# peterWon/LVI-ExC

Measured on AMD Instinct MI355X. Metric: M residual+Jacobian evals/s per GN iter, higher is better.
Workload: dtype f64; 1 GPU; config4-full-LVI: 1000000 surfel + 200000 IMU samples (gyro+accel blocks) + 49992 ORB reprojection blocks, 25023 knots @ dt=0.02; step = residuals + analytic Jacobians + Huber + J^T J/J^T r assembly (no linear solve); n_tangent=155259, bandwidth=179, n_border=52, tracks=orb, parallelism=sequence-per-gpu x1, allreduce_transport=none (one sequence)

## Files before the change

lvi-exc_amd/csrc/lvx_eval.hip:

```cpp
#include <algorithm>
#include <cmath>
#include <cstring>
#include <functional>
#include <numeric>
#include <cstdlib>

#include <thread>
#include "lvx_ctx.h"

namespace lvx {

#define LVX_PW 4
struct Keys { int k0, k1, lm; };
LVX_HD bool same(const Keys& a, const Keys& b) { return a.k0 == b.k0 && a.k1 == b.k1 && a.lm == b.lm; }

struct Cal { ImuCal imu; SensorCal lidar, cam; const double* rho; };
__device__ __forceinline__ Cal load_cal(const DevCommon& cm) {
  const double* s = cm.state + 7 * (size_t)cm.N;
  Cal c;
  c.imu.tau = s[7]; c.imu.roll = s[8]; c.imu.pitch = s[9]; c.imu.ba = load_v3(s + 10); c.imu.bg = load_v3(s + 13);
  c.lidar.q = load_q(s + 16); c.lidar.p = load_v3(s + 20); c.lidar.tau = s[23];
  c.cam.q = load_q(s + 24); c.cam.p = load_v3(s + 28); c.cam.tau = s[31];
  c.rho = s + 32;
  return c;
// ... 248 lines not shown
  double J[NR][NC];
  Keys key{-1, -1, -1};
  bool valid = false;
  if (in) {
    int status;
    if constexpr (EXP) status = eval_flat(fam, cm, sp, cal, hub, si, r, J, key);
    else status = fam.eval(cm, sp, cal, hub, si, r, J, key);
    valid = status == RES_OK;
    if (!valid) { atomicOr(cm.err, status); key = Keys{-1, -1, -1}; }
    if constexpr (EXP) {
      if (valid) put_record<NR, NC>(cm, F::FAM, fam.perm[si], key.k0, F::KEYS > 1 ? key.k1 : -1, F::KEYS > 2 ? key.lm : -1, [&](int a, int c) { return J[a][c]; });
      else put_skipped(cm, F::FAM, fam.perm[si]);
    }
  }
  double mycost = 0.0;
  if (valid) {
    double s = 0.0;
#pragma unroll
    for (int a = 0; a < NR; ++a) s += r[a] * r[a];
    double scale;
    mycost = 0.5 * huber_rho(fam.huber, s, &scale);
    const long long orow = row0 + (long long)fam.perm[si] * NR;
    if (cm.residuals) {
#pragma unroll
      for (int a = 0; a < NR; ++a) cm.residuals[orow + a] = r[a];
    }
    if (!EXP && cm.jcols) {
#pragma unroll
      for (int a = 0; a < NR; ++a) {
        int32_t* jc = cm.jcols + (orow + a) * LVX_JAC_WIDTH;
        double* jv = cm.jvals + (orow + a) * LVX_JAC_WIDTH;
#pragma unroll
        for (int c = 0; c < NC; ++c) {
          const int g = fam.col(c, key, cm.N);
          const bool dead = tangent_locked(g, cm.N, cm.L, cm.locks);
          jc[c] = dead ? -1 : g;
          jv[c] = dead ? 0.0 : J[a][c];
        }
        for (int c = NC; c < LVX_JAC_WIDTH; ++c) { jc[c] = -1; jv[c] = 0.0; }
      }
    }
    if (scale != 1.0) {
#pragma unroll
      for (int a = 0; a < NR; ++a) {
        r[a] *= scale;
#pragma unroll
        for (int c = 0; c < NC; ++c) J[a][c] *= scale;
      }
    }
  }
  mycost = wave_sum(mycost);
  if (lane == 0) atomicAdd(&cm.cost[rep], mycost);
  if (cm.what & LVX_EVAL_NORMAL_EQ) {
#pragma unroll
    for (int a = 0; a < NR; ++a) {
      rs[lane * NR + a] = valid ? r[a] : 0.0;
#pragma unroll
      for (int c = 0; c < NC; ++c) Jt[c * TS + lane * NR + a] = valid ? J[a][c] : 0.0;
    }
    Keys pk;
    pk.k0 = __shfl_up(key.k0, 1); pk.k1 = __shfl_up(key.k1, 1); pk.lm = __shfl_up(key.lm, 1);
    const bool head = (lane == 0) || !same(pk, key);
    const unsigned long long heads = __ballot(head);
    const int myseg = __popcll(heads & ((2ull << lane) - 1ull)) - 1;
    if (head) { seg_l0[myseg] = lane; seg_ok[myseg] = valid ? 1 : 0; seg_keys[myseg] = key; }
    if (lane == 0) nseg_s = __popcll(heads);
  }
  }
  if (!(cm.what & LVX_EVAL_NORMAL_EQ)) return;
  __syncthreads();
  const int nseg = nseg_s;
  const int tid = threadIdx.x;
  constexpr int NT = 64 * PW;
  for (int e = tid; e < nseg * NC; e += NT) { const int sg = e / NC, c = e % NC; cpos[e] = seg_ok[sg] ? cm.ord[fam.col(c, seg_keys[sg], cm.N)] : LVX_DEAD; }
  constexpr int ITER = (NP + NC + NT - 1) / NT;
  unsigned code[ITER];
#pragma unroll
  for (int i = 0; i < ITER; ++i) { const int p = tid + NT * i; code[i] = p < NP ? pairs[p] : 0u; }
  __syncthreads();
  for (int sg = 0; sg < nseg; ++sg) {
    if (!seg_ok[sg]) continue;
    const int l0 = seg_l0[sg];
    const int l1 = sg + 1 < nseg ? seg_l0[sg + 1] : 64;
    const int rb = l0 * NR, re = l1 * NR;
    const int* cp = &cpos[sg * NC];
#pragma unroll
    for (int i = 0; i < ITER; ++i) {
      const int p = tid + NT * i;
      if (p < NP) {
        const int a = code[i] & 0xff, b = code[i] >> 8;
        const int pa = cp[a], pb = cp[b];
        if (pa == LVX_DEAD || pb == LVX_DEAD) continue;
        const double* ja = &Jt[a * TS];
        const double* jb = &Jt[b * TS];
        double acc = 0.0;
        for (int row = rb; row < re; ++row) acc += ja[row] * jb[row];
        if (a != b && pa == pb) acc *= 2.0;
        add_H(cm, pa, pb, acc, rep);
      } else if (p < NP + NC) {
        const int c = p - NP;
        const int pc = cp[c];
        if (pc == LVX_DEAD) continue;
        const double* jc = &Jt[c * TS];
        double acc = 0.0;
        for (int row = rb; row < re; ++row) acc += jc[row] * rs[row];
        add_g(cm, pc, acc, rep);
      }
    }
  }
}

__device__ void hub_eval_thread(const DevCommon& cm, double t_map, int want_surf, int want_cs, HubShared* hubs, int s) {
  if (s > 1) return;
  if ((s == 0 && !want_surf) || (s == 1 && !want_cs)) { hubs[s].ok = 0; return; }
  const SplineRef sp{cm.t0, cm.dt, cm.N, cm.state, cm.state + 3 * (size_t)cm.N};
  const Cal cal = load_cal(cm);
  const bool tl = s == 0 ? (cm.locks & LVX_LOCK_LIDAR_TAU) != 0 : (cm.locks & LVX_LOCK_CAM_TAU) != 0;
  const double tau = s == 0 ? cal.lidar.tau : cal.cam.tau;
  double s1[1][2]; hub_spans(t_map, tl, cm.sensor_mto, s1);
  Segs sg; KnotRef kh; hubs[s].ok = 0;
  if (!build_segments(sp, s1, 1, &sg)) return;
  if (!seg_lookup(sp, sg, t_map + tau, &kh)) return;
  if (!(tl ? pose_eval<true>(sp, kh, &hubs[s].A) : pose_eval<true, true>(sp, kh, &hubs[s].A))) { hubs[s].ok = -RES_NONUNIT; return; }
  hub_matrix(hubs[s].A, hubs[s].M);
  hubs[s].ok = 1;
}
__device__ __forceinline__ void state_prepass_block(const DevCommon& cm, So3Pre* tab, int nblk_tab, double t_map, int want_surf, int want_cs, HubShared* hubs, int blk) {
  if (blk >= nblk_tab) { hub_eval_thread(cm, t_map, want_surf, want_cs, hubs, threadIdx.x); return; }
  const int k = blk * blockDim.x + threadIdx.x;
  if (k >= cm.N) return;
  const double* so3 = cm.state + 3 * (size_t)cm.N;
  So3Pre e;
  if (k + 1 < cm.N) so3_pre(load_q(so3 + 4 * (size_t)k), load_q(so3 + 4 * (size_t)(k + 1)), &e);
  else { e.Om = mk(0, 0, 0); e.on = 0.0; e.Jri = m3_identity(); e.c3 = 1.0 / 12.0; e.ok = 1; }
  tab[k] = e;
}

struct Aux { int wid, xk, lm; const PreWin* pw; };
struct GyroAcc {
  enum { PMAJ = 1 };
  enum { NK = 12, NG = 3, NR = 3, HUB = -1, KPK = 3, LVO = 3, WS = 1, GL = 32, SKIP_GG = 0, SECONDARY = 0, LB = 64, NCP = 15, USE_PRE = 1, OCC = 1, FAM = LVX_FAM_GYRO };
  __device__ static constexpr int jm(int c) { return c; }
  int n; const double* t; const double* m3; const int* perm; double weight, huber;
  __device__ int eval(const DevCommon& cm, const SplineRef& sp, const Cal& cal, const HubShared*, int si, double r[NR], double (*J)[NCP], int& key, Aux& aux) const {
    return gyro_residual<true, true>(sp, cal.imu, t[si], load_v3(m3 + 3 * (size_t)si), weight, &key, r, J, aux.pw);
  }
  __device__ static int klv(int c) { return 6 * (c / 3) + 3 + c % 3; }
  __device__ static int gcol(int g, int N, int nt) { return 6 * N + 5 + g; }
  __device__ void put(const DevCommon& cm, const HubShared*, int si, bool valid, int key, const double (*J)[NCP]) const {
    if (!valid) { put_skipped(cm, FAM, perm[si]); return; }
    put_record<NR, GYRO_NC>(cm, FAM, perm[si], key, -1, -1, [&](int a, int c) { return J[a][c]; });
  }
};
template <bool TAU> struct SurfAccT {
  enum { NK = 24, NG = 12 + (TAU ? 1 : 0), NR = 1, HUB = 0, KPK = 6, LVO = 0, WS = 2, GL = 16, SKIP_GG = 0, SECONDARY = 0, LB = 64, NCP = 36 + (TAU ? 1 : 0), USE_PRE = 1, OCC = 2, FAM = LVX_FAM_SURFEL };
  __device__ static constexpr int jm(int c) { return c; }
  int n; const double* t; const double* pt; const double* rowpl; const int* perm; double t_map, weight, huber;
  struct Row { double t; v3 p, Pi; };
  enum { PREFETCH = 1 };
  __device__ Row load(int si) const { return Row{t[si], load_v3(pt + 3 * (size_t)si), load_v3(rowpl + 3 * (size_t)si)}; }
  __device__ int eval_row(const DevCommon& cm, const SplineRef& sp, const Cal& cal, const HubShared* hub, const Row& row, double r[NR], double (*J)[NCP], int& key, Aux& aux) const {
    const bool tl = (cm.locks & LVX_LOCK_LIDAR_TAU) != 0;
    const double tk = row.t;
    Segs segs;
    if (tl) {
      KnotRef kr;
      const int st = two_point_lookup(sp, t_map, tk, tk + cal.lidar.tau, &kr);
      if (st >= 0) {
        if (st == 1) return RES_RANGE;
        if (hub->ok != 1) return hub->ok < 0 ? RES_NONUNIT : RES_RANGE;
        if (st == 2) return RES_RANGE;
        LVX_KT(aux.pw, 8)
        return surfel_residual_pseudo<true, TAU>(sp, hub->A, segs, cal.lidar, tk, row.p, row.Pi, weight, &key, r, J, aux.pw, &kr);
      }
    }
    const double pad = tl ? 0.0 : cm.sensor_mto;
    const double spans[2][2] = {{t_map - pad, t_map + pad}, {tk - pad, tk + pad}};
    if (!build_segments(sp, spans, 2, &segs)) return RES_RANGE;
    KnotRef kh;
    if (!seg_lookup(sp, segs, t_map + cal.lidar.tau, &kh)) return RES_RANGE;
    if (hub->ok != 1) return hub->ok < 0 ? RES_NONUNIT : RES_RANGE;
    if (kh.i0 != hub->A.k.i0 || kh.u != hub->A.k.u) return LVX_ERR_FALLBACK;
    LVX_KT(aux.pw, 8)
    return surfel_residual_pseudo<true, TAU>(sp, hub->A, segs, cal.lidar, tk, row.p, row.Pi, weight, &key, r, J, aux.pw);
  }
  __device__ static int klv(int c) { return c; }
  __device__ static int gcol(int g, int N, int nt) { return g < 6 ? nt + g : 6 * N + 8 + (g - 6); }
  __device__ void put(const DevCommon& cm, const HubShared* hub, int si, bool valid, int key, const double (*J)[NCP]) const {
    if (!valid) { put_skipped(cm, FAM, perm[si]); return; }
    put_record<NR, SURF_NC + (TAU ? 1 : 0)>(cm, FAM, perm[si], hub->A.k.i0, key, -1, [&](int a, int c) { return c < 24 ? hub_col(*hub, &J[a][24], c) : (c < 48 ? J[a][c - 24] : J[a][c - 18]); });
  }
};
using SurfAcc = SurfAccT<false>;
template <bool TAU> struct CamSurfAccT {
  enum { NK = 24, NG = 18 + (TAU ? 1 : 0), NR = 1, HUB = 1, KPK = 6, LVO = 0, WS = 1, GL = 16, SKIP_GG = 0, SECONDARY = 0, LB = 64, NCP = 42 + (TAU ? 1 : 0), USE_PRE = 1, OCC = 2, FAM = LVX_FAM_CAMSURF };
  __device__ static constexpr int jm(int c) { return c; }
  int n; const int* lm; const int* plane; const int* perm; const double* planes; const double* lm_uv; const double* lm_t0; double t_map, weight, huber;
  __device__ int eval(const DevCommon& cm, const SplineRef& sp, const Cal& cal, const HubShared* hub, int si, double r[NR], double (*J)[NCP], int& key, Aux& aux) const {
    const bool tl = (cm.locks & LVX_LOCK_CAM_TAU) != 0;
    const int l = lm[si];
    const double tk = lm_t0[l];
    Segs segs;
    if (tl) {
      KnotRef kr;
      const int st = two_point_lookup(sp, t_map, tk, tk + cal.cam.tau, &kr);
      if (st >= 0) {
        if (st == 1) return RES_RANGE;
        if (hub->ok != 1) return hub->ok < 0 ? RES_NONUNIT : RES_RANGE;
        if (st == 2) return RES_RANGE;
        return camsurf_residual_pseudo<true, TAU>(sp, hub->A, segs, cm.cam, cal.cam, cal.lidar, lm_uv[2 * l], lm_uv[2 * l + 1], tk, cal.rho[l],
                                                  load_v3(planes + 3 * (size_t)plane[si]), weight, &key, r, J, aux.pw, &kr);
      }
    }
    const double pad = tl ? 0.0 : cm.sensor_mto;
    const double spans[2][2] = {{t_map - pad, t_map + pad}, {tk - pad, tk + pad}};
    if (!build_segments(sp, spans, 2, &segs)) return RES_RANGE;
    KnotRef kh;
    if (!seg_lookup(sp, segs, t_map + cal.cam.tau, &kh)) return RES_RANGE;
    if (hub->ok != 1) return hub->ok < 0 ? RES_NONUNIT : RES_RANGE;
    if (kh.i0 != hub->A.k.i0 || kh.u != hub->A.k.u) return LVX_ERR_FALLBACK;
    return camsurf_residual_pseudo<true, TAU>(sp, hub->A, segs, cm.cam, cal.cam, cal.lidar, lm_uv[2 * l], lm_uv[2 * l + 1], tk, cal.rho[l],
                                              load_v3(planes + 3 * (size_t)plane[si]), weight, &key, r, J, aux.pw);
  }
  __device__ static int klv(int c) { return c; }
  __device__ static int gcol(int g, int N, int nt) { return g < 6 ? nt + 6 + g : (g < 12 ? 6 * N + 15 + (g - 6) : (g < 18 ? 6 * N + 8 + (g - 12) : 6 * N + 21)); }
  __device__ void put(const DevCommon& cm, const HubShared* hub, int si, bool valid, int key, const double (*J)[NCP]) const {
    if (!valid) { put_skipped(cm, FAM, perm[si]); return; }
    put_record<NR, CS_NC + (TAU ? 1 : 0)>(cm, FAM, perm[si], hub->A.k.i0, key, -1, [&](int a, int c) { return c < 24 ? hub_col(*hub, &J[a][24], c) : (c < 48 ? J[a][c - 24] : J[a][c - 18]); });
  }
};
using CamSurfAcc = CamSurfAccT<false>;

struct RepJac { const double* J; const double* r; const int* k; int n; };
template <int SIDE, bool TAU = false> struct RepSideAcc {
  enum { PMAJ = 1 };
  enum { NK = 24, NG = 6 + (TAU ? 1 : 0), NR = 2, HUB = -1, KPK = 6, LVO = 0, WS = 1, GL = 16, SKIP_GG = SIDE, SECONDARY = 1, LB = 16, NCP = 31 + (TAU ? 1 : 0), USE_PRE = 0, OCC = 1, FAM = LVX_FAM_REPROJ };
  __device__ static constexpr int jm(int c) { return c; }
  static constexpr int RJ = REP_NC + (TAU ? 1 : 0);
  int n; RepJac jac;
  double huber;
  __device__ int eval(const DevCommon&, const SplineRef&, const Cal&, const HubShared*, int si, double r[NR], double (*J)[NCP], int& key, Aux& aux) const {
    const int k = jac.k[(size_t)SIDE * jac.n + si];
    if (jac.k[(size_t)jac.n + si] < 0) return -1;
    key = k; aux.wid = k;
#pragma unroll
    for (int a = 0; a < 2; ++a) {
      r[a] = jac.r[(size_t)a * jac.n + si];
#pragma unroll
      for (int c = 0; c < 24; ++c) J[a][c] = jac.J[(size_t)(a * RJ + 24 * SIDE + c) * jac.n + si];
#pragma unroll
      for (int c = 0; c < 6; ++c) J[a][24 + c] = jac.J[(size_t)(a * RJ + 48 + c) * jac.n + si];
      if (TAU) J[a][30] = jac.J[(size_t)(a * RJ + 55) * jac.n + si];
    }
    return RES_OK;
  }
  __device__ static int gcol(int g, int N, int nt) { return 6 * N + 15 + g; }
};

template <bool TAU, bool EXP = false>
__global__ __launch_bounds__(64) void k_reproj_jac(ReprojFamT<TAU> fam, DevCommon cm, double* Jb, double* rb, int* kb, long long row0, double* Trec) {
  constexpr int RJ = REP_NC + (TAU ? 1 : 0), RW = 56 + (TAU ? 1 : 0);
  constexpr int RS = RW | 1;
  extern __shared__ double trec_s[];
  const int lane = threadIdx.x, si = blockIdx.x * 64 + lane, n = fam.n;
  const int rep = blockIdx.x % cm.nrep;
  double mycost = 0.0;
  if (si < n) {
    const SplineRef sp{cm.t0, cm.dt, cm.N, cm.state, cm.state + 3 * (size_t)cm.N};
    const Cal cal = load_cal(cm);
    HubShared none;
    double r[2], J[2][RJ];
    Keys key{-1, -1, -1};
    const int status = fam.eval_pre(cm, sp, cal, si, r, J, key);
    if constexpr (EXP) {
      if (status != RES_OK) put_skipped(cm, LVX_FAM_REPROJ, fam.perm[si]);
      else put_record<2, RJ>(cm, LVX_FAM_REPROJ, fam.perm[si], key.k0, key.k1, key.lm, [&](int a, int c) { return J[a][c]; });
    }
    if (status != RES_OK) { if (status == RES_OUTSIDE) fallback_row(cm, LVX_FAM_REPROJ, si); else atomicOr(cm.err, status); kb[si] = -1; kb[n + si] = -1; }
    else {
      double scale;
      mycost = 0.5 * huber_rho(fam.huber, r[0] * r[0] + r[1] * r[1], &scale);
      if (cm.residuals) { const long long orow = row0 + (long long)fam.perm[si] * 2; cm.residuals[orow] = r[0]; cm.residuals[orow + 1] = r[1]; }
      kb[si] = key.k0; kb[n + si] = key.k1;
      if (cm.what & LVX_EVAL_NORMAL_EQ) {
#pragma unroll
        for (int a = 0; a < 2; ++a) {
          rb[(size_t)a * n + si] = r[a] * scale;
#pragma unroll
          for (int c = 0; c < RJ; ++c) Jb[(size_t)(a * RJ + c) * n + si] = J[a][c] * scale;
        }
        if (Trec) {
          double* rec = trec_s + lane * RS;
          const double j0 = J[0][54] * scale, j1 = J[1][54] * scale;
#pragma unroll
          for (int c = 0; c < 54; ++c) rec[c] = j0 * (J[0][c] * scale) + j1 * (J[1][c] * scale);
          rec[54] = j0 * j0 + j1 * j1;
          rec[55] = j0 * (r[0] * scale) + j1 * (r[1] * scale);
          if (TAU) rec[56] = j0 * (J[0][55] * scale) + j1 * (J[1][55] * scale);
        }
      }
    }
  }
  if (Trec && (cm.what & LVX_EVAL_NORMAL_EQ)) {
    __builtin_amdgcn_fence(__ATOMIC_RELEASE, "wavefront");
    __builtin_amdgcn_wave_barrier();
    __builtin_amdgcn_fence(__ATOMIC_ACQUIRE, "wavefront");
    const int nrec = min(64, n - (int)blockIdx.x * 64);
    double* dst = Trec + (size_t)blockIdx.x * 64 * RW;
// ... 193 lines not shown
      else if (status != RES_OK) atomicOr(cm.err, status);
      else {
        valid = true;
        double scale;
        mycost = 0.5 * huber_rho(fam.huber, r[0] * r[0] + r[1] * r[1], &scale);
        if (cm.residuals) { const long long orow = row0 + (long long)fam.perm[si] * 2; cm.residuals[orow] = r[0]; cm.residuals[orow + 1] = r[1]; }
        if (scale != 1.0) {
#pragma unroll
          for (int a = 0; a < 2; ++a) {
            r[a] *= scale;
#pragma unroll
            for (int c = 0; c < RJ; ++c) J[a][c] *= scale;
          }
        }
      }
    }
    mycost = wave_sum(mycost);
    if (lane == 0 && mycost != 0.0) atomicAdd(&cm.cost[rep], mycost);
#ifdef RF_EVAL_ONLY
    if (cm.N > 0) continue;
#endif
    if (!want_ne) continue;
    const int my_w0 = valid ? key.k0 >> 2 : -1, my_w1 = valid ? key.k1 >> 2 : -1;
    const int my_o0 = 6 * (key.k0 & 3), my_o1 = 48 + 6 * (key.k1 & 3);
    const int my_p0 = (valid && lm_free) ? cm.lm_p0[key.lm] : 0;
    unsigned long long rem = __ballot(valid);
    while (rem) {
      const int lf = __ffsll((long long)rem) - 1;
      const int w0 = __builtin_amdgcn_readfirstlane(__shfl(my_w0, lf)), w1 = __builtin_amdgcn_readfirstlane(__shfl(my_w1, lf));
      const unsigned long long wm = __ballot(valid && my_w0 == w0 && my_w1 == w1);
      rem &= ~wm;
      for (int c = lane; c < 96; c += 64) {
        int tg = -1;
        if (c < 42) { if (4 * w0 + c / 6 < N) tg = 24 * w0 + c; }
        else if (c < 48) tg = 6 * N + 15 + (c - 42);
        else if (c < 90) { if (4 * w1 + (c - 48) / 6 < N) tg = 24 * w1 + (c - 48); }
        else if (c == TCOL && TAU) tg = 6 * N + 21;
        posL[c] = tg >= 0 ? cm.ord[tg] : LVX_DEAD;
      }
      d4 D[21];
#pragma unroll
      for (int t = 0; t < 21; ++t) D[t] = d4{0.0, 0.0, 0.0, 0.0};
      unsigned long long todo = wm;
      while (todo) {
        const int l0 = __ffsll((long long)todo) - 1;
        const int ws = min(l0, 48);
        const unsigned long long chunk = todo & (0xffffull << ws);
        todo &= ~chunk;
        for (int e = lane; e < 32 * LDP; e += 64) P[e] = 0.0;
        __builtin_amdgcn_fence(__ATOMIC_RELEASE, "wavefront");
        __builtin_amdgcn_wave_barrier();
        if ((chunk >> lane) & 1ull) {
#pragma unroll
          for (int a = 0; a < 2; ++a) {
            double* prow_ = P + ((lane - ws) * 2 + a) * LDP;
#pragma unroll
            for (int c = 0; c < 24; ++c) prow_[my_o0 + c] = J[a][c];
#pragma unroll
            for (int c = 0; c < 6; ++c) prow_[42 + c] = J[a][48 + c];
#pragma unroll
            for (int c = 0; c < 24; ++c) prow_[my_o1 + c] = J[a][24 + c];
            if (TAU) prow_[TCOL] = J[a][RJ - 1];
            prow_[RCOL] = r[a];
            prow_[LCOL] = J[a][54];
          }
        }
        __builtin_amdgcn_fence(__ATOMIC_RELEASE, "wavefront");
        __builtin_amdgcn_wave_barrier();
        __builtin_amdgcn_fence(__ATOMIC_ACQUIRE, "wavefront");
#ifndef RF_NO_LM
        if (lm_free) {
          for (int e0 = 0; e0 < 16 * (LCOL + 1); e0 += 64) {
            const int e = e0 + lane;
            const int li = min(e / (LCOL + 1), 15), c = e - li * (LCOL + 1);
            const int src = ws + li;
            const int p0 = __shfl(my_p0, src), l = __shfl(key.lm, src);
            if (e >= 16 * (LCOL + 1) || !((chunk >> src) & 1ull)) continue;
            const double* ra = P + (2 * li) * LDP;
            const double v = ra[LCOL] * ra[c] + ra[LDP + LCOL] * ra[LDP + c];
            if (v == 0.0) continue;
            int slot;
            if (c == RCOL) slot = cm.lm_wl + cm.nbd + 1;
            else if (c == LCOL) slot = cm.lm_wl + cm.nbd;
            else {
              const int p = posL[c];
              if (p == LVX_DEAD) continue;
              if (p >= 0) { slot = p - p0; if (slot < 0 || slot >= cm.lm_wl) { atomicOr(cm.err, 4); continue; } }
              else slot = cm.lm_wl + (-1 - p);
            }
            atomicAdd(&cm.lmH[(size_t)l * cm.lm_ls + slot], v);
          }
        }
#endif
        const int lhi = 63 - __clzll((long long)chunk);
        const int ks0 = (l0 - ws) >> 1, ks1 = (2 * (lhi - ws + 1) + 3) >> 2;
#ifndef RF_NO_MFMA
        for (int ks = ks0; ks < ks1; ++ks) {
          double f[6];
          const double* src = P + (4 * ks + (lane >> 4)) * LDP + (lane & 15);
#pragma unroll
          for (int c = 0; c < 6; ++c) f[c] = src[c * 16];
          int t = 0;
#pragma unroll
          for (int ci = 0; ci < 6; ++ci)
#pragma unroll
            for (int cj = ci; cj < 6; ++cj, ++t) D[t] = __builtin_amdgcn_mfma_f64_16x16x4f64(f[ci], f[cj], D[t], 0, 0, 0);
        }
#endif
        __builtin_amdgcn_fence(__ATOMIC_RELEASE, "wavefront");
        __builtin_amdgcn_wave_barrier();
      }
#pragma unroll
      for (int h = 0; h < 2; ++h) {
#pragma unroll
        for (int t = 11 * h; t < (h ? 21 : 11); ++t)
#pragma unroll
          for (int v = 0; v < 4; ++v) P[(t - 11 * h) * 256 + ((lane >> 4) + 4 * v) * 16 + (lane & 15)] = D[t][v];
        __builtin_amdgcn_fence(__ATOMIC_RELEASE, "wavefront");
        __builtin_amdgcn_wave_barrier();
        __builtin_amdgcn_fence(__ATOMIC_ACQUIRE, "wavefront");
#ifndef RF_NO_FLUSH
        for (int ci = 0, t = 0; ci < 6; ++ci)
          for (int cj = ci; cj < 6; ++cj, ++t) {
            if (t / 11 != h) continue;
            for (int e = lane; e < 256; e += 64) {
              const int row = ci * 16 + (e >> 4), col = cj * 16 + (e & 15);
              const double val = P[(t - 11 * h) * 256 + e];
              if (val == 0.0 || col < row) continue;
              const int pa = posL[row], pb = posL[col];
              if (row == RCOL) { if (col != RCOL && pb != LVX_DEAD) add_g(cm, pb, val, rep); continue; }
              if (col == RCOL) { if (pa != LVX_DEAD) add_g(cm, pa, val, rep); continue; }
              if (pa == LVX_DEAD || pb == LVX_DEAD) continue;
              add_H(cm, pa, pb, (pa == pb && row != col) ? 2.0 * val : val, rep);
            }
          }
#endif
        __builtin_amdgcn_fence(__ATOMIC_RELEASE, "wavefront");
        __builtin_amdgcn_wave_barrier();
      }
    }
  }
}

#define ACC_BW 24


struct NoRow {};
template <class F, class = void> struct RowOf { using type = NoRow; static constexpr bool prefetch = false; };
template <class F> struct RowOf<F, std::void_t<typename F::Row>> { using type = typename F::Row; static constexpr bool prefetch = true; };

template <class F, class = void> struct PanelMajor { static constexpr bool on = false; };
template <class F> struct PanelMajor<F, std::enable_if_t<(F::PMAJ > 0)>> { static constexpr bool on = true; static_assert(F::WS == 1, "panel-major needs shift-free windows"); };

template <class F> struct MfmaGeom {
  static constexpr int NKL = (F::WS + 3) * F::KPK;
  static constexpr int NCL = NKL + F::NG + 1;
  static constexpr int NT = (NCL + 15) / 16;
  static constexpr int LDP = (NT * 16) | 1;
  static constexpr int PR = F::GL * F::NR;
  static_assert(PR % 4 == 0, "panel rows must be a multiple of the MFMA k-step");
  static constexpr int NTP = NT * (NT + 1) / 2;
};
template <class F> size_t mfma_lds_bytes(int cr) {
  const int LV = (cr + 5) * 6;
  return (size_t)(LV * ACC_BW + F::NG * LV + F::NG * F::NG + LV + F::NG + 64 + 4 * MfmaGeom<F>::PR * MfmaGeom<F>::LDP) * 8 + (F::USE_PRE ? (size_t)(cr + 4) * sizeof(So3Pre) : 0) +
         (size_t)(LV + F::NG) * 4 + 64;
}

template <class F, int OCC, bool EXP = false>
__global__ __launch_bounds__(256, OCC) void k_family_mfma(F fam, DevCommon cm, const int* __restrict__ chunk_off, long long row0, int CR, int var_nch, const int* __restrict__ det_list) {
  using G = MfmaGeom<F>;
  constexpr int NK = F::NK, NG = F::NG, NC = F::NCP, NR = F::NR, KPK = F::KPK, WS = F::WS, GL = F::GL, LB = F::LB;
  constexpr int NKL = G::NKL, NT = G::NT, LDP = G::LDP, PR = G::PR;
  const int ACC_LV = (CR + 5) * 6;
  extern __shared__ double sm[];
  double* acc_band = sm;
  double* acc_bd = acc_band + ACC_LV * ACC_BW;
  double* acc_gg = acc_bd + NG * ACC_LV;
  double* acc_gk = acc_gg + NG * NG;
  double* acc_gG = acc_gk + ACC_LV;
  const int dummy = (int)(acc_gG + NG - sm);
  double* panels = acc_gG + NG + 64;
  So3Pre* pre_tab = (So3Pre*)(panels + 4 * PR * LDP);
  int* kpos = (int*)(pre_tab + (F::USE_PRE ? CR + 4 : 0));
  int* gpos = kpos + ACC_LV;
  const int tid = threadIdx.x, lane = tid & 63, wv = tid >> 6;
  const int ch = det_list ? det_list[blockIdx.x] : blockIdx.x;
  const int nwv = det_list ? 1 : 4;
  const int m0 = chunk_off[ch], m1 = chunk_off[ch + 1];
  if (m0 >= m1) return;
#ifdef LVX_KTIME
  long long kt_[16] = {0, 0, 0, 0, 0, 0, 0, 0, 0, 0, 0, 0, 0, 0, 0, 0}; long long kt0_ = __builtin_amdgcn_s_memtime(), kts_ = kt0_;
#define KT(i) { const long long n_ = __builtin_amdgcn_s_memtime(); kt_[i] += n_ - kt0_; kt0_ = n_; }
#else
#define KT(i)
#endif
  const int k_lo = (var_nch ? chunk_off[var_nch + 1 + ch] : ch * CR) - 1;
  const int nt = 6 * cm.N + 22 + cm.L;
  const bool want_ne = (cm.what & LVX_EVAL_NORMAL_EQ) != 0;
  const int LVU = var_nch ? min(ACC_LV, (chunk_off[2 * var_nch + 1 + ch] + 6) * 6) : ACC_LV;
  for (int e = tid; e < LVU * ACC_BW; e += 256) acc_band[e] = 0.0;
  for (int g = 0; g < NG; ++g) for (int e = tid; e < LVU; e += 256) acc_bd[g * ACC_LV + e] = 0.0;
  for (int e = tid; e < NG * NG + LVU; e += 256) { if (e < NG * NG) acc_gg[e] = 0.0; else acc_gk[e - NG * NG] = 0.0; }
  if (tid < NG) acc_gG[tid] = 0.0;
  for (int e = tid; e < 4 * PR * LDP; e += 256) panels[e] = 0.0;
  for (int e = tid; e < LVU; e += 256) { const int k = k_lo + e / 6; kpos[e] = (k >= 0 && k < cm.N) ? cm.ord[6 * k + e % 6] : LVX_DEAD; }
  if (tid < NG) gpos[tid] = cm.ord[F::gcol(tid, cm.N, nt)];
  const SplineRef sp{cm.t0, cm.dt, cm.N, cm.state, cm.state + 3 * (size_t)cm.N};
  if (F::USE_PRE && tid < CR + 4) {
    const int ka = k_lo + tid;
    if (ka >= 0 && ka + 1 < cm.N) pre_tab[tid] = cm.pre[ka];
    else { pre_tab[tid].Om = mk(0, 0, 0); pre_tab[tid].on = 0.0; pre_tab[tid].Jri = m3_identity(); pre_tab[tid].c3 = 1.0 / 12.0; pre_tab[tid].ok = 1; }
  }
#ifdef LVX_KTIME
  const PreWin pwin{pre_tab, k_lo, CR + 4, kt_};
#else
  const PreWin pwin{pre_tab, k_lo, CR + 4};
#endif
  const Cal cal = load_cal(cm);
  const HubShared* hub = F::HUB >= 0 ? ((const HubShared*)cm.hubs) + F::HUB : nullptr;
  double* P = panels + wv * (PR * LDP);
  const int rep = ch % cm.nrep;
  auto cls = [](int lc) { return lc < NKL ? 6 * (lc / KPK) + F::LVO + lc % KPK : (lc < NKL + NG ? -1 - (lc - NKL) : (lc == NKL + NG ? -100 : -200)); };
  const int frag_off = (lane >> 4) * LDP + (lane & 15);
  double mycost = 0.0;
  int rtab[PanelMajor<F>::on ? G::NTP * 4 : 1];
  if constexpr (PanelMajor<F>::on) {
    int t = 0;
#pragma unroll
    for (int ci = 0; ci < NT; ++ci)
#pragma unroll
      for (int cj = ci; cj < NT; ++cj, ++t)
#pragma unroll
        for (int v = 0; v < 4; ++v) {
          const int row = ci * 16 + (lane >> 4) + 4 * v, col = cj * 16 + (lane & 15);
          int ent = -1;
          if (!(ci == cj && col < row)) {
            const int ra = cls(row), cb = cls(col);
            if (ra >= 0) {
              if (cb >= 0) { const int d = cb - ra; if (d >= 0 && d < ACC_BW) ent = ((int)(acc_band - sm) + ra * ACC_BW + d) | (2 << 16) | (cb << 18); }
              else if (cb > -100) ent = ((int)(acc_bd - sm) + (-1 - cb) * ACC_LV + ra) | (1 << 16) | (ra << 18);
              else if (cb == -100) ent = ((int)(acc_gk - sm) + ra) | (1 << 16) | (ra << 18);
            } else if (ra > -100 && !F::SKIP_GG) {
              if (cb > -100 && cb < 0) ent = (int)(acc_gg - sm) + (-1 - ra) * NG + (-1 - cb);
              else if (cb == -100) ent = (int)(acc_gG - sm) + (-1 - ra);
            }
          }
          rtab[t * 4 + v] = ent;
        }
  }
  typename RowOf<F>::type nxt{};
  if constexpr (RowOf<F>::prefetch) { const int s0 = m0 + wv * LB + lane; if (wv < nwv && lane < LB && s0 < m1) nxt = fam.load(s0); }
  __syncthreads();
  KT(0)
  for (int base = wv < nwv ? m0 + wv * LB : m1; base < m1; base += nwv * LB) {
    const int si = base + lane;
    const bool in = lane < LB && si < m1;
    const typename RowOf<F>::type cur = nxt;
    double r[NR];
    double J[NR][NC];
    int key = -1;
    Aux aux{-1, 0, 0, &pwin};
    bool valid = false;
#ifdef LVX_KTIME
    kt_[15] = __builtin_amdgcn_s_memtime();
#endif
    if (in) {
      int status;
      if constexpr (RowOf<F>::prefetch) status = fam.eval_row(cm, sp, cal, hub, cur, r, J, key, aux);
      else status = fam.eval(cm, sp, cal, hub, si, r, J, key, aux);
      if (aux.wid < 0) aux.wid = key;
      valid = status == RES_OK;
      if (valid && (key < k_lo || key - k_lo > CR + 1 || 6 * (key - k_lo + 4) > LVU)) { valid = false; fallback_row(cm, F::FAM, si); }
      else if (!valid && status == LVX_ERR_FALLBACK) fallback_row(cm, F::FAM, si);
      else if (!valid && status > 0) atomicOr(cm.err, status);
    }
    if constexpr (RowOf<F>::prefetch) { const int sn = si + nwv * LB; if (lane < LB && sn < m1) nxt = fam.load(sn); }
    if constexpr (EXP) { if (in) fam.put(cm, hub, si, valid, key, J); }
    if (valid) {
      double s = 0.0;
#pragma unroll
      for (int a = 0; a < NR; ++a) s += r[a] * r[a];
      double scale;
      const double rho_s = huber_rho(fam.huber, s, &scale);
      if constexpr (!F::SECONDARY) {
        mycost += 0.5 * rho_s;
        if (cm.residuals) {
          const long long orow = row0 + (long long)fam.perm[si] * NR;
#pragma unroll
          for (int a = 0; a < NR; ++a) cm.residuals[orow + a] = r[a];
        }
      }
      if (scale != 1.0) {
#pragma unroll
        for (int a = 0; a < NR; ++a) {
          r[a] *= scale;
#pragma unroll
          for (int c = 0; c < NC; ++c) J[a][c] *= scale;
        }
      }
    }
    if (!want_ne) continue;
    KT(1)
    if constexpr (PanelMajor<F>::on) {
      const unsigned long long vm = __ballot(valid);
      for (int g0 = 0; g0 < LB; g0 += GL) {
        const unsigned long long pmask = (GL >= 64 ? ~0ull : ((1ull << GL) - 1ull)) << g0;
        unsigned long long rem = vm & pmask;
        if (!rem) continue;
        if (lane >= g0 && lane < g0 + GL) {
          const int li = lane - g0;
#pragma unroll
          for (int a = 0; a < NR; ++a) {
            double* prow = P + (li * NR + a) * LDP;
#pragma unroll
            for (int c = 0; c < NK; ++c) prow[c] = valid ? J[a][F::jm(c)] : 0.0;
#pragma unroll
            for (int g = 0; g < NG; ++g) prow[NKL + g] = valid ? J[a][F::jm(NK + g)] : 0.0;
            prow[NKL + NG] = valid ? r[a] : 0.0;
          }
        }
        __builtin_amdgcn_fence(__ATOMIC_RELEASE, "wavefront");
        __builtin_amdgcn_wave_barrier();
        __builtin_amdgcn_fence(__ATOMIC_ACQUIRE, "wavefront");
        KT(2)
        while (rem) {
          const int l0 = __ffsll((long long)rem) - 1;
          const int kw = __builtin_amdgcn_readfirstlane(__shfl(key, l0));
          const unsigned long long wm = __ballot(valid && key == kw) & pmask;
          rem &= ~wm;
          const int lhi = 63 - __clzll((long long)wm);
          const int wb = (kw - k_lo) * 6;
          const int r_lo = (l0 - g0) * NR, r_hi = (lhi - g0 + 1) * NR;
          const unsigned long long wsh = wm >> g0;
          d4 D[G::NTP];
#pragma unroll
          for (int t = 0; t < G::NTP; ++t) D[t] = d4{0.0, 0.0, 0.0, 0.0};
          const int nks = (r_hi - r_lo + 3) >> 2;
          const bool contig = __popcll(wm) == lhi - l0 + 1;
          auto trip = [&](int ks, auto UC) {
            constexpr int U = decltype(UC)::value;
            double f[U][NT];
#pragma unroll
            for (int q = 0; q < U; ++q) {
              const int rr = r_lo + 4 * (ks + q) + (lane >> 4);
              bool mine = rr < r_hi;
              if (!contig) mine = mine && ((wsh >> (rr / NR)) & 1ull);
              const double* src = P + min(rr, PR - 1) * LDP + (lane & 15);
#pragma unroll
              for (int c = 0; c < NT; ++c) { const double x = src[c * 16]; f[q][c] = mine ? x : 0.0; }
            }
#pragma unroll
            for (int q = 0; q < U; ++q) {
              int t = 0;
#pragma unroll
              for (int ci = 0; ci < NT; ++ci)
#pragma unroll
                for (int cj = ci; cj < NT; ++cj, ++t) D[t] = __builtin_amdgcn_mfma_f64_16x16x4f64(f[q][ci], f[q][cj], D[t], 0, 0, 0);
            }
          };
          int ks = 0;
          for (; ks + 6 <= nks; ks += 6) trip(ks, std::integral_constant<int, 6>{});
          for (; ks < nks; ks += 2) trip(ks, std::integral_constant<int, 2>{});
          KT(3)
          const int wbB = wb * ACC_BW;
#pragma unroll
          for (int t = 0; t < G::NTP; ++t)
#pragma unroll
            for (int v = 0; v < 4; ++v) {
              const int te = rtab[t * 4 + v];
              const bool ok = te >= 0 && wb + (te >> 18) < ACC_LV;
              const int m = (te >> 16) & 3;
              atomicAdd(&sm[ok ? (te & 0xffff) + (m == 2 ? wbB : (m == 1 ? wb : 0)) : dummy + lane], ok ? D[t][v] : 0.0);
            }
          KT(4)
        }
        __builtin_amdgcn_fence(__ATOMIC_RELEASE, "wavefront");
        __builtin_amdgcn_wave_barrier();
      }
      continue;
    }
    unsigned long long rem = __ballot(valid);
    while (rem) {
      const int l0 = __ffsll((long long)rem) - 1;
      const int kw = __builtin_amdgcn_readfirstlane(__shfl(key, l0));
      const int ww = __builtin_amdgcn_readfirstlane(__shfl(aux.wid, l0));
      const bool inw = valid && aux.wid >= ww && aux.wid < ww + WS && key >= kw && key < kw + WS;
      const unsigned long long wm = __ballot(inw);
      rem &= ~wm;
      const int lhi = 63 - __clzll((long long)wm);
      const int sh = inw ? (key - kw) * KPK : 0;
      const int wb = (kw - k_lo) * 6;
      d4 D[G::NTP];
#pragma unroll
      for (int t = 0; t < G::NTP; ++t) D[t] = d4{0.0, 0.0, 0.0, 0.0};
      for (int g0 = l0; g0 <= lhi; g0 += GL) {
        const int gs = min(g0, 64 - GL);
        if (lane >= gs && lane < gs + GL) {
          const int li = lane - gs;
          const bool mrow = inw && lane >= g0;
#pragma unroll
          for (int a = 0; a < NR; ++a) {
            double* prow = P + (li * NR + a) * LDP;
#pragma unroll
            for (int c = 0; c < NK; ++c) prow[sh + c] = mrow ? J[a][F::jm(c)] : 0.0;
#pragma unroll
            for (int z = 0; z < (WS - 1) * KPK; ++z) prow[z < sh ? z : z + NK] = 0.0;
#pragma unroll
            for (int g = 0; g < NG; ++g) prow[NKL + g] = mrow ? J[a][F::jm(NK + g)] : 0.0;
            prow[NKL + NG] = mrow ? r[a] : 0.0;
          }
        }
        __builtin_amdgcn_fence(__ATOMIC_RELEASE, "wavefront");
        __builtin_amdgcn_wave_barrier();
        __builtin_amdgcn_fence(__ATOMIC_ACQUIRE, "wavefront");
        KT(2)
        const int cnt = min(GL, lhi + 1 - gs);
        const int nks = (cnt * NR + 3) >> 2;
        for (int ks = 0; ks < nks; ++ks) {
          double f[NT];
#pragma unroll
          for (int c = 0; c < NT; ++c) f[c] = P[ks * 4 * LDP + frag_off + c * 16];
          int t = 0;
#pragma unroll
          for (int ci = 0; ci < NT; ++ci)
#pragma unroll
            for (int cj = ci; cj < NT; ++cj, ++t) D[t] = __builtin_amdgcn_mfma_f64_16x16x4f64(f[ci], f[cj], D[t], 0, 0, 0);
        }
        __builtin_amdgcn_fence(__ATOMIC_RELEASE, "wavefront");
        __builtin_amdgcn_wave_barrier();
        KT(3)
      }
      {
      int t = 0;
#pragma unroll
      for (int ci = 0; ci < NT; ++ci)
#pragma unroll
        for (int cj = ci; cj < NT; ++cj, ++t)
#pragma unroll
          for (int v = 0; v < 4; ++v) {
            const double val = D[t][v];
            if (val == 0.0) continue;
            if (ci == cj && (lane & 15) < (lane >> 4) + 4 * v) continue;
            const int ra = cls(ci * 16 + (lane >> 4) + 4 * v), cb = cls(cj * 16 + (lane & 15));
            if (ra >= 0) {
              const int la = wb + ra;
              if (la >= ACC_LV) continue;
              if (cb >= 0) { const int d = cb - ra; if (d < ACC_BW && wb + cb < ACC_LV) atomicAdd(&acc_band[la * ACC_BW + d], val); }
              else if (cb > -100) atomicAdd(&acc_bd[(-1 - cb) * ACC_LV + la], val);
              else if (cb == -100) atomicAdd(&acc_gk[la], val);
            } else if (ra > -100) {
              const int ga = -1 - ra;
              if (cb > -100) {
                const int gb = -1 - cb;
                if (!F::SKIP_GG) atomicAdd(&acc_gg[ga * NG + gb], val);
              } else if (cb == -100) {
                if (!F::SKIP_GG) atomicAdd(&acc_gG[ga], val);
              }
            }
          }
      }
      KT(4)
    }
  }
  if (!F::SECONDARY) {
    mycost = wave_sum(mycost);
    if (lane == 0) atomicAdd(&cm.cost[rep], mycost);
  }
  if (!want_ne) return;
  KT(5)
  __syncthreads();
  KT(6)
  for (int e = tid; e < LVU * ACC_BW; e += 256) {
    const double v = acc_band[e];
    if (v == 0.0) continue;
    const int la = e / ACC_BW, lb = la + e % ACC_BW;
    if (lb >= LVU) continue;
    const int pa = kpos[la], pb = kpos[lb];
    if (pa == LVX_DEAD || pb == LVX_DEAD) continue;
    add_H(cm, pa, pb, v, rep);
  }
  for (int g = 0; g < NG; ++g)
    for (int e = tid; e < LVU; e += 256) {
      const double v = acc_bd[g * ACC_LV + e];
      if (v == 0.0) continue;
      const int pg = gpos[g], pk2 = kpos[e];
      if (pg == LVX_DEAD || pk2 == LVX_DEAD) continue;
      add_H(cm, pg, pk2, v, rep);
    }
  for (int e = tid; e < NG * NG; e += 256) {
    const int ga = e / NG, gb2 = e % NG;
    if (gb2 < ga) continue;
    const double v = acc_gg[e];
    if (v == 0.0 || gpos[ga] == LVX_DEAD || gpos[gb2] == LVX_DEAD) continue;
    add_H(cm, gpos[ga], gpos[gb2], v, rep);
  }
  for (int e = tid; e < LVU; e += 256) { const double v = acc_gk[e]; if (v != 0.0 && kpos[e] != LVX_DEAD) add_g(cm, kpos[e], v, rep); }
  if (tid < NG) { const double v = acc_gG[tid]; if (v != 0.0 && gpos[tid] != LVX_DEAD) add_g(cm, gpos[tid], v, rep); }
#ifdef LVX_KTIME
  KT(7)
#ifndef LVX_KTIME_FAM
#define LVX_KTIME_FAM SurfAcc
#endif
  if (std::is_same<F, LVX_KTIME_FAM>::value && lane == 0 && blockIdx.x % (gridDim.x / 8 + 1) == 5)
    printf("KT wg %d wv %d rows %d CR %d: init %lld eval %lld [seg %lld lookup %lld value %lld chain %lld pull %lld] panel %lld mfma %lld wflush %lld tail %lld sync %lld flush %lld total %lld\n", (int)blockIdx.x, wv, m1 - m0, CR,
           kt_[0], kt_[1], kt_[8], kt_[9], kt_[10], kt_[11], kt_[12], kt_[2], kt_[3], kt_[4], kt_[5], kt_[6], kt_[7], (long long)__builtin_amdgcn_s_memtime() - kts_);
#endif
}

struct ImuG { enum { NR = 3, NCJ = GYRO_NC, NK = 12, NG = 3, KPK = 3, LVO = 3, GL = 32, GOFF = 5, NKL = 12, NCL = 16, NT = 1, NTP = 1, LDP = 18, PR = 96 }; };
struct ImuA { enum { NR = 3, NCJ = ACC_NC, NK = 24, NG = 5, KPK = 6, LVO = 0, GL = 16, GOFF = 0, NKL = 24, NCL = 30, NT = 2, NTP = 3, LDP = 34, PR = 48 }; };
#define IMU_NGA 8
struct ImuAccLds { double* band; double* bd; double* gg; double* gk; double* gG; int lv; };
template <class PG> __device__ __forceinline__ int imu_cls(int lc) {
  return lc < PG::NKL ? 6 * (lc / PG::KPK) + PG::LVO + lc % PG::KPK : (lc < PG::NKL + PG::NG ? -1 - (PG::GOFF + lc - PG::NKL) : (lc == PG::NKL + PG::NG ? -100 : -200));
}
template <class PG> __device__ __forceinline__ void imu_build_rtab(int* rtab, int lane, const double* sm, const ImuAccLds& A) {
  int t = 0;
#pragma unroll
  for (int ci = 0; ci < PG::NT; ++ci)
#pragma unroll
    for (int cj = ci; cj < PG::NT; ++cj, ++t)
#pragma unroll
      for (int v = 0; v < 4; ++v) {
        const int row = ci * 16 + (lane >> 4) + 4 * v, col = cj * 16 + (lane & 15);
        int ent = -1;
        if (!(ci == cj && col < row)) {
          const int ra = imu_cls<PG>(row), cb = imu_cls<PG>(col);
          if (ra >= 0) {
            if (cb >= 0) { const int d = cb - ra; if (d >= 0 && d < ACC_BW) ent = ((int)(A.band - sm) + ra * ACC_BW + d) | (2 << 16) | (cb << 18); }
            else if (cb > -100) ent = ((int)(A.bd - sm) + (-1 - cb) * A.lv + ra) | (1 << 16) | (ra << 18);
            else if (cb == -100) ent = ((int)(A.gk - sm) + ra) | (1 << 16) | (ra << 18);
          } else if (ra > -100) {
            if (cb > -100 && cb < 0) ent = (int)(A.gg - sm) + (-1 - ra) * IMU_NGA + (-1 - cb);
            else if (cb == -100) ent = (int)(A.gG - sm) + (-1 - ra);
          }
        }
        rtab[t * 4 + v] = ent;
      }
}
template <class PG> __device__ __forceinline__ void imu_assemble(double* sm, double* P, const int* rtab, bool valid, int key, int k_lo, int acc_lv, const double* r, const double (*J)[PG::NCJ], int lane, int dummy) {
  constexpr int NR = PG::NR, NT = PG::NT, LDP = PG::LDP, PR = PG::PR, GL = PG::GL;
  const unsigned long long vm = __ballot(valid);
  for (int g0 = 0; g0 < 64; g0 += GL) {
    const unsigned long long pmask = ((1ull << GL) - 1ull) << g0;
    unsigned long long rem = vm & pmask;
    if (!rem) continue;
    if (lane >= g0 && lane < g0 + GL) {
      const int li = lane - g0;
#pragma unroll
      for (int a = 0; a < NR; ++a) {
        double2* prow2 = (double2*)(P + (li * NR + a) * LDP);
        auto col = [&](int c) { return c < PG::NK + PG::NG ? (valid ? J[a][c] : 0.0) : (c == PG::NK + PG::NG ? (valid ? r[a] : 0.0) : 0.0); };
#pragma unroll
        for (int c2 = 0; c2 < 8 * NT; ++c2) prow2[c2] = make_double2(col(2 * c2), col(2 * c2 + 1));
      }
    }
    __builtin_amdgcn_fence(__ATOMIC_RELEASE, "wavefront");
    __builtin_amdgcn_wave_barrier();
    __builtin_amdgcn_fence(__ATOMIC_ACQUIRE, "wavefront");
    while (rem) {
      const int l0 = __ffsll((long long)rem) - 1;
      const int kw = __builtin_amdgcn_readfirstlane(__shfl(key, l0));
      const unsigned long long wm = __ballot(valid && key == kw) & pmask;
      rem &= ~wm;
      const int lhi = 63 - __clzll((long long)wm);
      const int wb = (kw - k_lo) * 6;
      const int r_lo = (l0 - g0) * NR, r_hi = (lhi - g0 + 1) * NR;
      const unsigned long long wsh = wm >> g0;
      const bool contig = __popcll(wm) == lhi - l0 + 1;
      d4 D[PG::NTP];
#pragma unroll
      for (int t = 0; t < PG::NTP; ++t) D[t] = d4{0.0, 0.0, 0.0, 0.0};
      const int nks = (r_hi - r_lo + 3) >> 2;
      auto trip = [&](int ks, auto UC) {
        constexpr int U = decltype(UC)::value;
        double f[U][NT];
#pragma unroll
        for (int q = 0; q < U; ++q) {
          const int rr = r_lo + 4 * (ks + q) + (lane >> 4);
          bool mine = rr < r_hi;
          if (!contig) mine = mine && ((wsh >> (rr / NR)) & 1ull);
          const double* src = P + min(rr, PR - 1) * LDP + (lane & 15);
#pragma unroll
          for (int c = 0; c < NT; ++c) { const double x = src[c * 16]; f[q][c] = mine ? x : 0.0; }
        }
#pragma unroll
        for (int q = 0; q < U; ++q) {
          int t = 0;
#pragma unroll
          for (int ci = 0; ci < NT; ++ci)
#pragma unroll
            for (int cj = ci; cj < NT; ++cj, ++t) D[t] = __builtin_amdgcn_mfma_f64_16x16x4f64(f[q][ci], f[q][cj], D[t], 0, 0, 0);
        }
      };
      int ks = 0;
      for (; ks + 6 <= nks; ks += 6) trip(ks, std::integral_constant<int, 6>{});
      for (; ks < nks; ks += 2) trip(ks, std::integral_constant<int, 2>{});
      const int wbB = wb * ACC_BW;
#pragma unroll
      for (int t = 0; t < PG::NTP; ++t)
#pragma unroll
        for (int v = 0; v < 4; ++v) {
          const int te = rtab[t * 4 + v];
          const bool ok = te >= 0 && wb + (te >> 18) < acc_lv;
          const int m = (te >> 16) & 3;
          const int idx = ok ? (te & 0xffff) + (m == 2 ? wbB : (m == 1 ? wb : 0)) : dummy + lane;
          atomicAdd(&sm[idx], ok ? D[t][v] : 0.0);
        }
    }
    __builtin_amdgcn_fence(__ATOMIC_RELEASE, "wavefront");
    __builtin_amdgcn_wave_barrier();
  }
}
struct ImuFused { int n; const double* t; const double* gyro; const double* acc; const int* perm; double w_gyro, w_acc; };
#define IMU_CR 32
#define IMU_LV ((IMU_CR + 5) * 6)
struct ImuOwn { const int* wg_c0; const int* own_k; int nch, span; };
#define LVX_LDS_BARRIER() asm volatile("s_waitcnt lgkmcnt(0)\n\ts_barrier" ::: "memory")
static size_t imu_fused_lds_bytes(int span) {
  const int pan = std::max((int)ImuG::PR * (int)ImuG::LDP, (int)ImuA::PR * (int)ImuA::LDP);
  return (size_t)(IMU_LV * ACC_BW + IMU_NGA * IMU_LV + IMU_NGA * IMU_NGA + IMU_LV + IMU_NGA + 64 + 4 * pan) * 8 + (size_t)span * sizeof(So3Pre) + (size_t)(7 * span + IMU_NGA) * 4 + 64;
}
__global__ void k_imu_rtab(int* out) {
  const int lane = threadIdx.x;
  const double* sm = (const double*)out;
  ImuAccLds A;
  A.band = (double*)sm; A.bd = A.band + IMU_LV * ACC_BW; A.gg = A.bd + IMU_NGA * IMU_LV; A.gk = A.gg + IMU_NGA * IMU_NGA; A.gG = A.gk + IMU_LV; A.lv = IMU_LV;
  int rtg[ImuG::NTP * 4], rta[ImuA::NTP * 4];
  imu_build_rtab<ImuG>(rtg, lane, sm, A);
  imu_build_rtab<ImuA>(rta, lane, sm, A);
  for (int i = 0; i < ImuG::NTP * 4; ++i) out[i * 64 + lane] = rtg[i];
  for (int i = 0; i < ImuA::NTP * 4; ++i) out[(ImuG::NTP * 4 + i) * 64 + lane] = rta[i];
}
template <bool EXP = false>
__global__ __launch_bounds__(256, 1) void k_imu_own(ImuFused fam, DevCommon cm, const int* __restrict__ chunk_off, ImuOwn ow, long long row0_g, long long row0_a, int det, const int* __restrict__ rtab_g) {
  constexpr int PAN = (ImuG::PR * ImuG::LDP > ImuA::PR * ImuA::LDP) ? ImuG::PR * ImuG::LDP : ImuA::PR * ImuA::LDP;
  constexpr int ACC_LV = IMU_LV, CR = IMU_CR, HB = ACC_BW / 2;
  extern __shared__ __attribute__((aligned(16))) double smo[];
  double* sm = smo;
  ImuAccLds A;
  A.band = sm; A.bd = A.band + ACC_LV * ACC_BW; A.gg = A.bd + IMU_NGA * ACC_LV; A.gk = A.gg + IMU_NGA * IMU_NGA; A.gG = A.gk + ACC_LV; A.lv = ACC_LV;
  double* panels = A.gG + IMU_NGA + 64;
  So3Pre* pre_all = (So3Pre*)(panels + 4 * PAN);
  int* kpos_all = (int*)(pre_all + ow.span);
  int* kown_all = kpos_all + 6 * ow.span;
  int* gpos = kown_all + ow.span;
  const int tid = threadIdx.x, lane = tid & 63, wv = tid >> 6;
  const int wg = blockIdx.x;
  const int c0 = ow.wg_c0[wg], c1 = ow.wg_c0[wg + 1];
  if (c0 >= c1) return;
// ... 1438 lines not shown
```

Before: 2683 Mevals/s.

## Derive surfel dependent global Jacobian columns from knot blocks and widen window

For the surfel family, the first three global columns are treated as linear combinations (negated sums) of the knot translation columns. They are dropped from the MFMA panel, which narrows the column count and the number of tiles, and their Hessian/gradient blocks are rebuilt after accumulation by summing band entries. The surfel window shift is also raised from 2 to 3, which widens the knot panel. The intent is to cut MFMA work and panel traffic per row. The cost is extra reduction work in the flush stage and an added block barrier, and the result is only correct if the dependence identity holds exactly.

```diff
diff --git a/lvi-exc_amd/csrc/lvx_eval.hip b/lvi-exc_amd/csrc/lvx_eval.hip
--- a/lvi-exc_amd/csrc/lvx_eval.hip
+++ b/lvi-exc_amd/csrc/lvx_eval.hip
@@ -424,8 +424,12 @@
     put_record<NR, GYRO_NC>(cm, FAM, perm[si], key, -1, -1, [&](int a, int c) { return J[a][c]; });
   }
 };
+#ifndef LVX_SURF_WS
+#define LVX_SURF_WS 3
+#endif
 template <bool TAU> struct SurfAccT {
-  enum { NK = 24, NG = 12 + (TAU ? 1 : 0), NR = 1, HUB = 0, KPK = 6, LVO = 0, WS = 2, GL = 16, SKIP_GG = 0, SECONDARY = 0, LB = 64, NCP = 36 + (TAU ? 1 : 0), USE_PRE = 1, OCC = 2, FAM = LVX_FAM_SURFEL };
+  enum { DEPG = LVX_SURF_WS >= 3 ? 3 : 0 };
+  enum { NK = 24, NG = 12 + (TAU ? 1 : 0), NR = 1, HUB = 0, KPK = 6, LVO = 0, WS = LVX_SURF_WS, GL = 16, SKIP_GG = 0, SECONDARY = 0, LB = 64, NCP = 36 + (TAU ? 1 : 0), USE_PRE = 1, OCC = 2, FAM = LVX_FAM_SURFEL };
   __device__ static constexpr int jm(int c) { return c; }
   int n; const double* t; const double* pt; const double* rowpl; const int* perm; double t_map, weight, huber;
   struct Row { double t; v3 p, Pi; };
@@ -925,9 +929,14 @@
 template <class F, class = void> struct PanelMajor { static constexpr bool on = false; };
 template <class F> struct PanelMajor<F, std::enable_if_t<(F::PMAJ > 0)>> { static constexpr bool on = true; static_assert(F::WS == 1, "panel-major needs shift-free windows"); };
 
+template <class F, class = void> struct DepGlobals { static constexpr int n = 0; };
+template <class F> struct DepGlobals<F, std::enable_if_t<(F::DEPG > 0)>> { static constexpr int n = F::DEPG; };
+
 template <class F> struct MfmaGeom {
+  static constexpr int DEPG = DepGlobals<F>::n;
+  static constexpr int NGP = F::NG - DEPG;
   static constexpr int NKL = (F::WS + 3) * F::KPK;
-  static constexpr int NCL = NKL + F::NG + 1;
+  static constexpr int NCL = NKL + NGP + 1;
   static constexpr int NT = (NCL + 15) / 16;
   static constexpr int LDP = (NT * 16) | 1;
   static constexpr int PR = F::GL * F::NR;
@@ -944,7 +953,7 @@
 __global__ __launch_bounds__(256, OCC) void k_family_mfma(F fam, DevCommon cm, const int* __restrict__ chunk_off, long long row0, int CR, int var_nch, const int* __restrict__ det_list) {
   using G = MfmaGeom<F>;
   constexpr int NK = F::NK, NG = F::NG, NC = F::NCP, NR = F::NR, KPK = F::KPK, WS = F::WS, GL = F::GL, LB = F::LB;
-  constexpr int NKL = G::NKL, NT = G::NT, LDP = G::LDP, PR = G::PR;
+  constexpr int NKL = G::NKL, NT = G::NT, LDP = G::LDP, PR = G::PR, DEPG = G::DEPG, NGP = G::NGP;
   const int ACC_LV = (CR + 5) * 6;
   extern __shared__ double sm[];
   double* acc_band = sm;
@@ -994,7 +1003,7 @@
   const HubShared* hub = F::HUB >= 0 ? ((const HubShared*)cm.hubs) + F::HUB : nullptr;
   double* P = panels + wv * (PR * LDP);
   const int rep = ch % cm.nrep;
-  auto cls = [](int lc) { return lc < NKL ? 6 * (lc / KPK) + F::LVO + lc % KPK : (lc < NKL + NG ? -1 - (lc - NKL) : (lc == NKL + NG ? -100 : -200)); };
+  auto cls = [](int lc) { return lc < NKL ? 6 * (lc / KPK) + F::LVO + lc % KPK : (lc < NKL + NGP ? -1 - (DEPG + lc - NKL) : (lc == NKL + NGP ? -100 : -200)); };
   const int frag_off = (lane >> 4) * LDP + (lane & 15);
   double mycost = 0.0;
   int rtab[PanelMajor<F>::on ? G::NTP * 4 : 1];
@@ -1089,8 +1098,8 @@
 #pragma unroll
             for (int c = 0; c < NK; ++c) prow[c] = valid ? J[a][F::jm(c)] : 0.0;
 #pragma unroll
-            for (int g = 0; g < NG; ++g) prow[NKL + g] = valid ? J[a][F::jm(NK + g)] : 0.0;
-            prow[NKL + NG] = valid ? r[a] : 0.0;
+            for (int g = 0; g < NGP; ++g) prow[NKL + g] = valid ? J[a][F::jm(NK + DEPG + g)] : 0.0;
+            prow[NKL + NGP] = valid ? r[a] : 0.0;
           }
         }
         __builtin_amdgcn_fence(__ATOMIC_RELEASE, "wavefront");
@@ -1180,8 +1189,8 @@
 #pragma unroll
             for (int z = 0; z < (WS - 1) * KPK; ++z) prow[z < sh ? z : z + NK] = 0.0;
 #pragma unroll
-            for (int g = 0; g < NG; ++g) prow[NKL + g] = mrow ? J[a][F::jm(NK + g)] : 0.0;
-            prow[NKL + NG] = mrow ? r[a] : 0.0;
+            for (int g = 0; g < NGP; ++g) prow[NKL + g] = mrow ? J[a][F::jm(NK + DEPG + g)] : 0.0;
+            prow[NKL + NGP] = mrow ? r[a] : 0.0;
           }
         }
         __builtin_amdgcn_fence(__ATOMIC_RELEASE, "wavefront");
@@ -1253,7 +1262,7 @@
     if (pa == LVX_DEAD || pb == LVX_DEAD) continue;
     add_H(cm, pa, pb, v, rep);
   }
-  for (int g = 0; g < NG; ++g)
+  for (int g = DEPG; g < NG; ++g)
     for (int e = tid; e < LVU; e += 256) {
       const double v = acc_bd[g * ACC_LV + e];
       if (v == 0.0) continue;
@@ -1263,13 +1272,58 @@
     }
   for (int e = tid; e < NG * NG; e += 256) {
     const int ga = e / NG, gb2 = e % NG;
-    if (gb2 < ga) continue;
+    if (gb2 < ga || ga < DEPG) continue;
     const double v = acc_gg[e];
     if (v == 0.0 || gpos[ga] == LVX_DEAD || gpos[gb2] == LVX_DEAD) continue;
     add_H(cm, gpos[ga], gpos[gb2], v, rep);
   }
   for (int e = tid; e < LVU; e += 256) { const double v = acc_gk[e]; if (v != 0.0 && kpos[e] != LVX_DEAD) add_g(cm, kpos[e], v, rep); }
-  if (tid < NG) { const double v = acc_gG[tid]; if (v != 0.0 && gpos[tid] != LVX_DEAD) add_g(cm, gpos[tid], v, rep); }
+  if (tid >= DEPG && tid < NG) { const double v = acc_gG[tid]; if (v != 0.0 && gpos[tid] != LVX_DEAD) add_g(cm, gpos[tid], v, rep); }
+  if constexpr (DEPG > 0) {
+    const int nkn = LVU / 6;
+    auto ksum = [nkn](const double* src) {
+      double s = 0.0;
+      for (int k0 = 0; k0 < nkn; k0 += 8) {
+        double v[8];
+#pragma unroll
+        for (int j = 0; j < 8; ++j) v[j] = src[6 * min(k0 + j, nkn - 1)];
+#pragma unroll
+        for (int j = 0; j < 8; ++j) s += k0 + j < nkn ? v[j] : 0.0;
+      }
+      return -s;
+    };
+    for (int e = tid; e < DEPG * LVU; e += 256) {
+      const int b = e / LVU, la = e % LVU;
+      double v[9];
+#pragma unroll
+      for (int j = 0; j < 9; ++j) {
+        const int kk = la / 6 - 4 + j, c = 6 * kk + F::LVO + b, lo = min(c, la), d = max(c, la) - lo;
+        const bool ok = kk >= 0 && kk < nkn && d < ACC_BW;
+        v[j] = ok ? acc_band[ok ? lo * ACC_BW + d : 0] : 0.0;
+      }
+      double s = 0.0;
+#pragma unroll
+      for (int j = 0; j < 9; ++j) s += v[j];
+      acc_bd[b * ACC_LV + la] = -s;
+      if (s != 0.0 && gpos[b] != LVX_DEAD && kpos[la] != LVX_DEAD) add_H(cm, gpos[b], kpos[la], -s, rep);
+    }
+    const int q = 255 - tid;
+    if (q < DEPG * NGP) {
+      const int b = q / NGP, g = DEPG + q % NGP;
+      const double v = ksum(acc_bd + g * ACC_LV + F::LVO + b);
+      if (v != 0.0 && gpos[b] != LVX_DEAD && gpos[g] != LVX_DEAD) add_H(cm, gpos[b], gpos[g], v, rep);
+    } else if (q < DEPG * NGP + DEPG) {
+      const int b = q - DEPG * NGP;
+      const double v = ksum(acc_gk + F::LVO + b);
+      if (v != 0.0 && gpos[b] != LVX_DEAD) add_g(cm, gpos[b], v, rep);
+    }
+    __syncthreads();
+    if (tid < DEPG * DEPG && tid % DEPG >= tid / DEPG) {
+      const int b = tid / DEPG, b2 = tid % DEPG;
+      const double v = ksum(acc_bd + b * ACC_LV + F::LVO + b2);
+      if (v != 0.0 && gpos[b] != LVX_DEAD && gpos[b2] != LVX_DEAD) add_H(cm, gpos[b], gpos[b2], v, rep);
+    }
+  }
 #ifdef LVX_KTIME
   KT(7)
 #ifndef LVX_KTIME_FAM
```

After: 2750 Mevals/s, median of 6. 2.5% higher.
